# Nuralamsiddik16/Ultrafnd_git

Hardware: AMD Instinct MI355X
Metric: train-step samples/sec (FakeSV batch, seq128+224^2) (higher is better)
Workload: dtype bf16

## Files before the change

ultrafnd_git_amd/csrc/attn_softmax.hpp:

```cpp
#pragma once
#include "common.hpp"

#pragma clang fp contract(off)

__device__ __forceinline__ bf16x8 lds_frag(const char* tile, int row, int chunk) {
  return *reinterpret_cast<const bf16x8*>(tile + row * 128 + ((chunk ^ ((row >> 1) & 7)) << 4));
}

__device__ __forceinline__ bool masked_block_is_noop(const float* kb, int lane, const float (&m_run)[2]) {
  return __all(kb[lane] != 0.0f) && __all(m_run[0] > -1.0e30f && m_run[1] > -1.0e30f);
}

template <int KT, bool DROP = false, bool CAUSAL = false>
__device__ __forceinline__ float online_softmax_block(f32x4 (&s)[KT][2], const int qt, const float* kbias, const bool any_masked, const int g,
                                                      const float scale_log2e, float& m_run, float& l_run, bf16x8 (&pf)[KT / 2][2],
                                                      const f32x4* dm = nullptr, const int qk = 0, const float causal_neg = 0.0f) {
  float mx = -INFINITY, lsum = 0.0f, m_new, alpha;
  if (any_masked) {
#pragma unroll
    for (int kt = 0; kt < KT; ++kt) {
      const f32x4 kbv = *reinterpret_cast<const f32x4*>(kbias + kt * 16 + 4 * g);
#pragma unroll
      for (int r = 0; r < 4; ++r) {
        float v = (kbv[r] == 0.0f) ? s[kt][qt][r] * scale_log2e : kbv[r];
        if constexpr (CAUSAL) {
          if (kbv[r] == 0.0f && 16 * kt + r > qk) v = causal_neg;
        }
        s[kt][qt][r] = v;
        mx = fmaxf(mx, v);
      }
    }
    mx = fmaxf(mx, __shfl_xor(mx, 16, 64));
    mx = fmaxf(mx, __shfl_xor(mx, 32, 64));
    m_new = fmaxf(m_run, mx);
    alpha = fast_exp2(m_run - m_new);
#pragma unroll
    for (int kt = 0; kt < KT; ++kt)
#pragma unroll
      for (int r = 0; r < 4; ++r) {
        const float p = fast_exp2(s[kt][qt][r] - m_new);
        lsum += p;
        if constexpr (DROP) pf[kt >> 1][qt][(kt & 1) * 4 + r] = (__bf16)(p * dm[kt][r]);
        else pf[kt >> 1][qt][(kt & 1) * 4 + r] = (__bf16)p;
      }
  } else {
#pragma unroll
    for (int kt = 0; kt < KT; ++kt)
#pragma unroll
      for (int r = 0; r < 4; ++r) mx = fmaxf(mx, s[kt][qt][r]);
    mx = fmaxf(mx, __shfl_xor(mx, 16, 64));
    mx = fmaxf(mx, __shfl_xor(mx, 32, 64));
    m_new = fmaxf(m_run, mx * scale_log2e);
    alpha = fast_exp2(m_run - m_new);
    const float neg_m = -m_new;
#pragma unroll
    for (int kt = 0; kt < KT; ++kt)
#pragma unroll
      for (int r = 0; r < 4; ++r) {
        const float p = fast_exp2(__builtin_fmaf(s[kt][qt][r], scale_log2e, neg_m));
        lsum += p;
        if constexpr (DROP) pf[kt >> 1][qt][(kt & 1) * 4 + r] = (__bf16)(p * dm[kt][r]);
        else pf[kt >> 1][qt][(kt & 1) * 4 + r] = (__bf16)p;
      }
  }
  l_run = __builtin_fmaf(l_run, alpha, lsum);
  m_run = m_new;
  return alpha;
}

__device__ __forceinline__ void attn_init(f32x4 (&o)[4][2], float (&m_run)[2], float (&l_run)[2]) {
#pragma unroll
  for (int dt = 0; dt < 4; ++dt)
#pragma unroll
    for (int qt = 0; qt < 2; ++qt) o[dt][qt] = f32x4{0.f, 0.f, 0.f, 0.f};
#pragma unroll
  for (int qt = 0; qt < 2; ++qt) m_run[qt] = -INFINITY, l_run[qt] = 0.f;
}

template <class QRow>
__device__ __forceinline__ void attn_q_frags(const char* qimg, QRow q_row, int fr, int g, bf16x8 (&qf)[2][2]) {
#pragma unroll
  for (int qt = 0; qt < 2; ++qt) {
    const int row = q_row(qt * 16 + fr);
    qf[qt][0] = lds_frag(qimg, row, g);
    qf[qt][1] = lds_frag(qimg, row, g + 4);
  }
}

template <int KT, class KeyRow>
__device__ __forceinline__ void attn_scores(const char* kimg, KeyRow key_row, const bf16x8 (&qf)[2][2], int fr, int g, f32x4 (&s)[KT][2]) {
#pragma unroll
  for (int kt = 0; kt < KT; ++kt)
#pragma unroll
    for (int qt = 0; qt < 2; ++qt) s[kt][qt] = f32x4{0.f, 0.f, 0.f, 0.f};
#pragma unroll
  for (int kk = 0; kk < 2; ++kk)
#pragma unroll
    for (int kt = 0; kt < KT; ++kt) {
      const bf16x8 kf = lds_frag(kimg, key_row(kt * 16 + fr), g + 4 * kk);
#pragma unroll
      for (int qt = 0; qt < 2; ++qt) s[kt][qt] = __builtin_amdgcn_mfma_f32_16x16x32_bf16(kf, qf[qt][kk], s[kt][qt], 0, 0, 0);
    }
}

template <int KT, bool DROP = false, bool CAUSAL = false>
__device__ __forceinline__ void attn_softmax_rescale(f32x4 (&s)[KT][2], const int qt, const float* kbias, const bool any_masked, const int g,
                                                     const float scale_log2e, float (&m_run)[2], float (&l_run)[2], bf16x8 (&pf)[KT / 2][2],
                                                     f32x4 (&o)[4][2], const f32x4* dm = nullptr, const int qk = 0, const float causal_neg = 0.0f) {
  const float alpha = online_softmax_block<KT, DROP, CAUSAL>(s, qt, kbias, any_masked, g, scale_log2e, m_run[qt], l_run[qt], pf, dm, qk, causal_neg);
  if (!__all(alpha == 1.0f)) {
#pragma unroll
    for (int dt = 0; dt < 4; ++dt) o[dt][qt] *= alpha;
  }
}

template <int KT, class KeyRow>
__device__ __forceinline__ void attn_pv(const char* vimg, KeyRow key_row, const bf16x8 (&pf)[KT / 2][2], f32x4 (&o)[4][2], int fr, int g) {
#pragma unroll
  for (int ksd = 0; ksd < KT / 2; ++ksd) {
#pragma unroll
    for (int dt = 0; dt < 4; ++dt) {
      const int qq = fr >> 2, pp = fr & 3;
      const int k0 = 32 * ksd + 4 * g + qq;
      const int key0 = key_row(k0), key1 = key_row(k0 + 16);
      const int ch = 2 * dt + (pp >> 1);
      const int off0 = key0 * 128 + ((ch ^ (((key0 >> 1) & 3) << 1)) << 4) + 8 * (pp & 1);
      const int off1 = key1 * 128 + ((ch ^ (((key1 >> 1) & 3) << 1)) << 4) + 8 * (pp & 1);
      const s16x4 t0 = __builtin_amdgcn_ds_read_tr16_b64_v4i16((s16x4 __attribute__((address_space(3)))*)(vimg + off0));
      const s16x4 t1 = __builtin_amdgcn_ds_read_tr16_b64_v4i16((s16x4 __attribute__((address_space(3)))*)(vimg + off1));
      union { s16x4 s2[2]; bf16x8 v; } u;
      u.s2[0] = t0;
      u.s2[1] = t1;
#pragma unroll
      for (int qt = 0; qt < 2; ++qt) o[dt][qt] = __builtin_amdgcn_mfma_f32_16x16x32_bf16(u.v, pf[ksd][qt], o[dt][qt], 0, 0, 0);
    }
  }
}

__device__ __forceinline__ float attn_finish(const float l_run, float& l) {
  l = l_run;
  l += __shfl_xor(l, 16, 64);
  l += __shfl_xor(l, 32, 64);
  return 1.0f / l;
}
__device__ __forceinline__ float attn_finish(const float l_run) {
  float l;
  return attn_finish(l_run, l);
}

__device__ __forceinline__ void attn_store_ctx(__bf16* dst, const f32x4 (&o)[4][2], const int qt, const float inv) {
#pragma unroll
  for (int dt = 0; dt < 4; ++dt) {
    bf16x4 ov = {(__bf16)(o[dt][qt][0] * inv), (__bf16)(o[dt][qt][1] * inv), (__bf16)(o[dt][qt][2] * inv), (__bf16)(o[dt][qt][3] * inv)};
    *reinterpret_cast<bf16x4*>(dst + dt * 16) = ov;
  }
}
```

ultrafnd_git_amd/csrc/common.hpp:

```cpp
#pragma once
#include <hip/hip_runtime.h>
#include <stdint.h>
#include <stdio.h>

#include "../../include/ultrafnd_hip.h"

typedef float f32x16 __attribute__((ext_vector_type(16)));
typedef float f32x4 __attribute__((ext_vector_type(4)));
typedef float f32x2 __attribute__((ext_vector_type(2)));
typedef __bf16 bf16x8 __attribute__((ext_vector_type(8)));
typedef __bf16 bf16x4 __attribute__((ext_vector_type(4)));
typedef short s16x4 __attribute__((ext_vector_type(4)));

#define UFND_WAVE 64

void ufnd_set_error(const char* fmt, ...);
#define UFND_REQUIRE(cond, ...)                      \
  do {                                               \
    if (!(cond)) {                                   \
      ufnd_set_error(__VA_ARGS__);                   \
      return UFND_ERR_INVALID;                       \
    }                                                \
  } while (0)
#define UFND_CHECK_LAUNCH()                                              \
  do {                                                                   \
    hipError_t e_ = hipGetLastError();                                   \
    if (e_ != hipSuccess) {                                              \
      ufnd_set_error("%s:%d launch failed: %s", __FILE__, __LINE__,      \
                     hipGetErrorString(e_));                             \
      return UFND_ERR_LAUNCH;                                            \
    }                                                                    \
  } while (0)

static inline bool ufnd_aligned(const void* p, size_t a) { return (reinterpret_cast<uintptr_t>(p) % a) == 0; }
static inline int ufnd_cdiv(int a, int b) { return (a + b - 1) / b; }

__device__ __forceinline__ float gelu_f(float x) {
  return 0.5f * x * (1.0f + erff(x * 0.70710678118654752440f));
}
__device__ __forceinline__ float gelu_grad_f(float x) {
  const float cdf = 0.5f * (1.0f + erff(x * 0.70710678118654752440f));
  const float pdf = 0.39894228040143267794f * __expf(-0.5f * x * x);
  return cdf + x * pdf;
}
__device__ __forceinline__ float sigmoid_f(float x) { return 1.0f / (1.0f + __expf(-x)); }
__device__ __forceinline__ int xcd_contiguous_id(int n, int total) {
  const int q = total >> 3, r = total & 7, xcd = n & 7, idx = n >> 3;
  return (xcd < r ? xcd * (q + 1) : r * (q + 1) + (xcd - r) * q) + idx;
}

__device__ __forceinline__ float fast_exp2(float x) { return __builtin_amdgcn_exp2f(x); }
__device__ __forceinline__ float quick_gelu_grad_f(float x) {
  const float s = 1.0f / (1.0f + __expf(-1.702f * x));
  return s * (1.0f + 1.702f * x * (1.0f - s));
}
__device__ __forceinline__ float sigmoid_fast_f(float x) {
#pragma clang fp contract(off)
  return __builtin_amdgcn_rcpf(__fadd_rn(1.0f, __expf(-x)));
}
__device__ __forceinline__ float quick_gelu_fast_f(float x) {
#pragma clang fp contract(off)
  return __fmul_rn(x, sigmoid_fast_f(__fmul_rn(1.702f, x)));
}
__device__ __forceinline__ float gelu_fast_f(float x) {
#pragma clang fp contract(off)
  const float z = __fmul_rn(fabsf(x), 0.70710678118654752440f);
  const float t = __builtin_amdgcn_rcpf(__fmaf_rn(0.3275911f, z, 1.0f));
  float p = __fmaf_rn(t, 1.061405429f, -1.453152027f);
  p = __fmaf_rn(t, p, 1.421413741f);
  p = __fmaf_rn(t, p, -0.284496736f);
  p = __fmaf_rn(t, p, 0.254829592f);
  const float poly = __fmul_rn(t, p);
  const float erf_abs = __fmaf_rn(-poly, __expf(__fmul_rn(-z, z)), 1.0f);
  const float h = __fmul_rn(0.5f, x);
  return __fmaf_rn(h, copysignf(erf_abs, x), h);
}

__device__ __forceinline__ f32x2 gelu_fast_f2(f32x2 x) {
#pragma clang fp contract(off)
  const f32x2 z = __builtin_elementwise_abs(x) * 0.70710678118654752440f;
  const f32x2 u = __builtin_elementwise_fma(f32x2{0.3275911f, 0.3275911f}, z, f32x2{1.0f, 1.0f});
  const f32x2 t = {__builtin_amdgcn_rcpf(u.x), __builtin_amdgcn_rcpf(u.y)};
  f32x2 p = __builtin_elementwise_fma(t, f32x2{1.061405429f, 1.061405429f}, f32x2{-1.453152027f, -1.453152027f});
  p = __builtin_elementwise_fma(t, p, f32x2{1.421413741f, 1.421413741f});
  p = __builtin_elementwise_fma(t, p, f32x2{-0.284496736f, -0.284496736f});
  p = __builtin_elementwise_fma(t, p, f32x2{0.254829592f, 0.254829592f});
  const f32x2 poly = t * p;
  const f32x2 zz = (-z) * z;
  const f32x2 e = {__expf(zz.x), __expf(zz.y)};
  const f32x2 erf_abs = __builtin_elementwise_fma(-poly, e, f32x2{1.0f, 1.0f});
  const f32x2 h = x * 0.5f;
  const f32x2 sg = {copysignf(erf_abs.x, x.x), copysignf(erf_abs.y, x.y)};
  return __builtin_elementwise_fma(h, sg, h);
}
__device__ __forceinline__ f32x2 quick_gelu_fast_f2(f32x2 x) {
#pragma clang fp contract(off)
  const f32x2 m = x * 1.702f;
  const f32x2 d = f32x2{__expf(-m.x), __expf(-m.y)} + 1.0f;
  const f32x2 r = {__builtin_amdgcn_rcpf(d.x), __builtin_amdgcn_rcpf(d.y)};
  return x * r;
}

__device__ __forceinline__ float quad_xor1(float v) {
  return __builtin_bit_cast(float, __builtin_amdgcn_update_dpp(0, __builtin_bit_cast(int, v), 0xB1, 0xF, 0xF, false));
}
__device__ __forceinline__ float quad_xor2(float v) {
  return __builtin_bit_cast(float, __builtin_amdgcn_update_dpp(0, __builtin_bit_cast(int, v), 0x4E, 0xF, 0xF, false));
}

#define UFND_DPP(v, old, ctrl, rmask) \
  __builtin_bit_cast(float, __builtin_amdgcn_update_dpp(__builtin_bit_cast(int, (float)(old)), __builtin_bit_cast(int, (float)(v)), ctrl, rmask, 0xF, false))
__device__ __forceinline__ float wave_sum(float v) {
  v += UFND_DPP(v, 0.0f, 0xB1, 0xF);
  v += UFND_DPP(v, 0.0f, 0x4E, 0xF);
  v += UFND_DPP(v, 0.0f, 0x141, 0xF);
  v += UFND_DPP(v, 0.0f, 0x140, 0xF);
  v += UFND_DPP(v, 0.0f, 0x142, 0xA);
  v += UFND_DPP(v, 0.0f, 0x143, 0xC);
  return __builtin_bit_cast(float, __builtin_amdgcn_readlane(__builtin_bit_cast(int, v), 63));
}
__device__ __forceinline__ float wave_max(float v) {
  v = fmaxf(v, UFND_DPP(v, v, 0xB1, 0xF));
  v = fmaxf(v, UFND_DPP(v, v, 0x4E, 0xF));
  v = fmaxf(v, UFND_DPP(v, v, 0x141, 0xF));
  v = fmaxf(v, UFND_DPP(v, v, 0x140, 0xF));
  v = fmaxf(v, UFND_DPP(v, v, 0x142, 0xA));
  v = fmaxf(v, UFND_DPP(v, v, 0x143, 0xC));
  return __builtin_bit_cast(float, __builtin_amdgcn_readlane(__builtin_bit_cast(int, v), 63));
}

__device__ __forceinline__ void philox_4x32(uint64_t seed, uint64_t step, uint32_t layer, uint32_t ctr, uint32_t (&out)[4]) {
  uint32_t k0 = (uint32_t)seed, k1 = (uint32_t)(seed >> 32);
  uint32_t c0 = ctr, c1 = layer, c2 = (uint32_t)step, c3 = (uint32_t)(step >> 32);
#pragma unroll
  for (int r = 0; r < 10; ++r) {
    const uint64_t p0 = (uint64_t)0xD2511F53u * c0;
    const uint64_t p1 = (uint64_t)0xCD9E8D57u * c2;
    const uint32_t n0 = (uint32_t)(p1 >> 32) ^ c1 ^ k0;
    const uint32_t n1 = (uint32_t)p1;
    const uint32_t n2 = (uint32_t)(p0 >> 32) ^ c3 ^ k1;
    const uint32_t n3 = (uint32_t)p0;
    c0 = n0; c1 = n1; c2 = n2; c3 = n3;
    k0 += 0x9E3779B9u; k1 += 0xBB67AE85u;
  }
  out[0] = c0; out[1] = c1; out[2] = c2; out[3] = c3;
}
__device__ __forceinline__ float dropout_keep(uint32_t r, float p) {
  const float u = (float)(r >> 8) * (1.0f / 16777216.0f);
  return (u >= p) ? 1.0f / (1.0f - p) : 0.0f;
}
__device__ __forceinline__ uint64_t dropout_step_key(const ufnd_step_state* st) { return st->step + ((uint64_t)st->micro << 40); }
__device__ __forceinline__ float dropout_mul(const ufnd_step_state* st, float p, uint32_t layer, uint32_t elem) {
  if (p <= 0.0f) return 1.0f;
  uint32_t w[4];
  philox_4x32(st->seed, dropout_step_key(st), layer, elem >> 2, w);
  const uint32_t k = elem & 3u;
  return dropout_keep(k == 0 ? w[0] : (k == 1 ? w[1] : (k == 2 ? w[2] : w[3])), p);
}
__device__ __forceinline__ void dropout_mul4(const ufnd_step_state* st, float p, uint32_t layer, uint32_t elem4, float (&m)[4]) {
  if (p <= 0.0f) { m[0] = m[1] = m[2] = m[3] = 1.0f; return; }
  uint32_t w[4];
  philox_4x32(st->seed, dropout_step_key(st), layer, elem4 >> 2, w);
#pragma unroll
  for (int q = 0; q < 4; ++q) m[q] = dropout_keep(w[q], p);
}
__device__ __forceinline__ void dropout_mul4_ctr(uint64_t seed, uint64_t step, float p, uint32_t layer, uint32_t ctr, float (&m)[4]) {
  uint32_t w[4];
  philox_4x32(seed, step, layer, ctr, w);
#pragma unroll
  for (int q = 0; q < 4; ++q) m[q] = dropout_keep(w[q], p);
}

static inline bool ufnd_attn_dropout_fits(int B, int L, int heads) {
  const long long lp = (L + 3) / 4 * 4;
  return (long long)B * heads * L * lp / 4 <= (1ll << 32);
}
constexpr uint32_t UFND_TAG_TEXT = 256;
constexpr uint32_t UFND_TAG_VISION = 4096;
```

ultrafnd_git_amd/csrc/encoders.hip:

```cpp
#include "rowwise.hpp"

namespace {

template <int NI>
__global__ __launch_bounds__(256) void layernorm_kernel(const float* x, int ldx, const float* gamma, const float* beta,
                                                        __bf16* ob, float* of, int M, int H, float eps, const int* m_live) {
  const int lane = threadIdx.x & 63;
  const int row = blockIdx.x * 4 + (threadIdx.x >> 6);
  if (row >= M || (m_live && row >= *m_live)) return;
  f32x4 v[NI];
#pragma unroll
  for (int i = 0; i < NI; ++i) v[i] = ld4(x + (size_t)row * ldx + 4 * lane + 256 * i);
  ln_row<NI>(v, H, eps, gamma, beta, lane);
  store_row<NI>(v, ob, of, row, H, lane);
}

template <int NI, bool RESID>
__global__ __launch_bounds__(256) void dropout_layernorm_kernel(const float* x, int ldx, const float* d, int ldd, const float* gamma,
                                                                const float* beta, float* y, __bf16* ob, float* of, int M, int H, float eps,
                                                                ufnd_dropout dr) {
  const int lane = threadIdx.x & 63;
  const int row = blockIdx.x * 4 + (threadIdx.x >> 6);
  if (row >= M) return;
  const uint64_t seed = dr.state->seed, step = dropout_step_key(dr.state);
  f32x4 v[NI], m[NI];
#pragma unroll
  for (int i = 0; i < NI; ++i) {
    const int col = 4 * lane + 256 * i;
    float m4[4];
    dropout_mul4_ctr(seed, step, dr.p, dr.tag, (uint32_t)(((size_t)row * H + col) >> 2), m4);
    m[i] = f32x4{m4[0], m4[1], m4[2], m4[3]};
    v[i] = ld4(x + (size_t)row * ldx + col);
    if constexpr (RESID) {
      v[i] += m[i] * ld4(d + (size_t)row * ldd + col);
      *reinterpret_cast<f32x4*>(y + (size_t)row * H + col) = v[i];
    }
  }
  ln_row<NI>(v, H, eps, gamma, beta, lane);
  if constexpr (!RESID) {
#pragma unroll
    for (int i = 0; i < NI; ++i) v[i] *= m[i];
  }
  store_row<NI>(v, ob, of, row, H, lane);
}

template <int NI>
__global__ __launch_bounds__(256) void bert_embed_kernel(const int64_t* ids, const float* word, const float* pos,
                                                         const float* type0, const float* gamma, const float* beta,
                                                         __bf16* ob, float* of, int M, int L, int H, int vocab,
                                                         float eps, const int32_t* row_src, const int* m_live) {
  const int lane = threadIdx.x & 63;
  const int row = blockIdx.x * 4 + (threadIdx.x >> 6);
  if (row >= M || (m_live && row >= *m_live)) return;
  const int src = row_src ? row_src[row] : row;
  long long id = ids[src];
  id = id < 0 ? 0 : (id >= vocab ? vocab - 1 : id);
  int l = src % L;
  l = l < 0 ? 0 : (l >= L ? L - 1 : l);
  f32x4 v[NI];
#pragma unroll
  for (int i = 0; i < NI; ++i) {
    const int col = 4 * lane + 256 * i;
    v[i] = ld4(word + (size_t)id * H + col) + ld4(pos + (size_t)l * H + col) + ld4(type0 + col);
  }
  if (gamma) ln_row<NI>(v, H, eps, gamma, beta, lane);
  store_row<NI>(v, ob, of, row, H, lane);
}

template <bool PACKED>
__global__ __launch_bounds__(256) void meanpool_kernel(const float* hidden, const int32_t* mask, float* out, int L, int H, const int32_t* cu) {
  __shared__ f32x4 part[4][64];
  __shared__ float cnts[4];
  const int b = blockIdx.y, col = blockIdx.x * 256 + 4 * (threadIdx.x & 63), grp = threadIdx.x >> 6, lane = threadIdx.x & 63;
  f32x4 acc = {0.f, 0.f, 0.f, 0.f};
  float cnt = 0.0f;
  const size_t r0 = PACKED ? (size_t)cu[b] : (size_t)b * L;
  const int n = PACKED ? cu[b + 1] - cu[b] : L;
  for (int l0 = grp; l0 < n; l0 += 32) {
    int mk[8];
    f32x4 x[8];
#pragma unroll
    for (int u = 0; u < 8; ++u) {
      const int l = l0 + 4 * u;
      mk[u] = l < n ? mask[(size_t)b * L + l] : 0;
    }
#pragma unroll
    for (int u = 0; u < 8; ++u) {
      const int l = l0 + 4 * u < n ? l0 + 4 * u : n - 1;
      x[u] = ld4(hidden + (r0 + l) * H + col);
    }
#pragma unroll
    for (int u = 0; u < 8; ++u) {
      if (mk[u] != 0) {
        acc += x[u];
        cnt += 1.0f;
      }
    }
  }
  part[grp][lane] = acc;
  if (lane == 0) cnts[grp] = cnt;
  __syncthreads();
  if (grp == 0) {
    const f32x4 s = (part[0][lane] + part[1][lane]) + (part[2][lane] + part[3][lane]);
    const float denom = fmaxf((cnts[0] + cnts[1]) + (cnts[2] + cnts[3]), 1e-6f);
    *reinterpret_cast<f32x4*>(out + (size_t)b * H + col) = s / denom;
  }
}
template <int NI>
__global__ __launch_bounds__(256) void ln_meanpool_kernel(const float* y, const float* gamma, const float* beta, float eps, const int32_t* mask,
                                                          const int32_t* cu, float* out, int L, int H) {
  __shared__ f32x4 part[4][NI][64];
  __shared__ float cnts[4];
  const int b = blockIdx.x, grp = __builtin_amdgcn_readfirstlane(threadIdx.x >> 6), lane = threadIdx.x & 63;
  const size_t r0 = (size_t)cu[b];
  const int n = cu[b + 1] - cu[b];
  f32x4 acc[NI];
#pragma unroll
  for (int i = 0; i < NI; ++i) acc[i] = f32x4{0.f, 0.f, 0.f, 0.f};
  float cnt = 0.0f;
  for (int l0 = grp; l0 < n; l0 += 32) {
    int mk[8];
    f32x4 v[8][NI];
#pragma unroll
    for (int u = 0; u < 8; ++u) {
      const int l = l0 + 4 * u;
      mk[u] = l < n ? mask[(size_t)b * L + l] : 0;
    }
#pragma unroll
    for (int u = 0; u < 8; ++u) {
      const int l = l0 + 4 * u < n ? l0 + 4 * u : n - 1;
#pragma unroll
      for (int i = 0; i < NI; ++i) v[u][i] = ld4(y + (r0 + l) * H + 4 * lane + 256 * i);
    }
#pragma unroll
    for (int u = 0; u < 8; ++u) ln_row<NI>(v[u], H, eps, gamma, beta, lane);
#pragma unroll
    for (int u = 0; u < 8; ++u) {
      if (mk[u] != 0) {
#pragma unroll
        for (int i = 0; i < NI; ++i) acc[i] += v[u][i];
        cnt += 1.0f;
      }
    }
  }
#pragma unroll
  for (int i = 0; i < NI; ++i) part[grp][i][lane] = acc[i];
  if (lane == 0) cnts[grp] = cnt;
  __syncthreads();
  if (grp == 0) {
    const float denom = fmaxf((cnts[0] + cnts[1]) + (cnts[2] + cnts[3]), 1e-6f);
#pragma unroll
    for (int i = 0; i < NI; ++i) {
      const f32x4 s = (part[0][i][lane] + part[1][i][lane]) + (part[2][i][lane] + part[3][i][lane]);
      *reinterpret_cast<f32x4*>(out + (size_t)b * H + 4 * lane + 256 * i) = s / denom;
    }
  }
}

__device__ __forceinline__ void pack_slot_bins(const int* lens, int total, int B, int32_t* bins, int32_t* nbins) {
  __shared__ long long csum[PACK_THREADS / 64];
  const int tid = threadIdx.x, wave = tid >> 6, lane = tid & 63;
  const int per = (B + PACK_THREADS - 1) / PACK_THREADS, b0 = tid * per, b1 = min(b0 + per, B);
  auto nrows = [&](int b) { return (b + 1 < B ? lens[b + 1] : total) - lens[b]; };
  long long cown = 0;
  for (int b = b0; b < b1; ++b) {
    const int c = (nrows(b) + 31) >> 5;
    if (c > 0) cown += 1ll << (16 * (c - 1));
  }
  long long cinc = cown;
#pragma unroll
  for (int o = 1; o < 64; o <<= 1) {
    const long long y = __shfl_up(cinc, o, 64);
    if (lane >= o) cinc += y;
  }
  if (lane == 63) csum[wave] = cinc;
  __syncthreads();
  long long cbase = 0, call = 0;
  for (int w = 0; w < PACK_THREADS / 64; ++w) {
    if (w < wave) cbase += csum[w];
    call += csum[w];
  }
  auto field = [](long long v, int c) { return (int)((v >> (16 * (c - 1))) & 0xffff); };
  const int n1 = field(call, 1), n2 = field(call, 2), n3 = field(call, 3), n4 = field(call, 4);
  const int p = min(n1, n3), r1 = n1 - p, h = n2 >> 1, t = n2 & 1, u = t ? min(2, r1) : 0;
  const bool odd_full = t && u == 2;
  const int f1 = (r1 - u) >> 2, rem1 = (r1 - u) & 3;
  const int b31 = n4, b22 = b31 + p, b211 = b22 + h, b1111 = b211 + (odd_full ? 1 : 0);
  const int bp3 = b1111 + f1, bp2 = bp3 + (n3 - p), bp1 = bp2 + ((t && !odd_full) ? 1 : 0), nb = bp1 + (rem1 ? 1 : 0);
  const int bodd = odd_full ? b211 : bp2;
  long long rank = cbase + cinc - cown;
  for (int b = b0; b < b1; ++b) {
    const int n = nrows(b), c = (n + 31) >> 5;
    if (c == 0) continue;
    const int k = field(rank, c);
    rank += 1ll << (16 * (c - 1));
    int bin, s0;
    if (c == 4) {
      bin = k, s0 = 0;
    } else if (c == 3) {
      bin = k < p ? b31 + k : bp3 + (k - p), s0 = 0;
    } else if (c == 2) {
      bin = k < 2 * h ? b22 + (k >> 1) : bodd, s0 = k < 2 * h ? 2 * (k & 1) : 0;
    } else if (k < p) {
      bin = b31 + k, s0 = 3;
    } else if (k - p < u) {
      bin = bodd, s0 = 2 + (k - p);
    } else {
      const int k1 = k - p - u;
      bin = (k1 >> 2) < f1 ? b1111 + (k1 >> 2) : bp1, s0 = k1 & 3;
    }
    for (int s = 0; s < c; ++s) {
      bins[(size_t)bin * 8 + 2 * (s0 + s)] = lens[b] + 32 * s;
      bins[(size_t)bin * 8 + 2 * (s0 + s) + 1] = (b << 10) | (s << 8) | n;
    }
  }
  for (int i = bp3 + tid; i < nb; i += PACK_THREADS) {
    const int used = i < bp2 ? 3 : (i < bp1 ? 2 + u : rem1);
    for (int j = used; j < 4; ++j) {
      bins[(size_t)i * 8 + 2 * j] = 0;
      bins[(size_t)i * 8 + 2 * j + 1] = -1;
    }
  }
  if (tid == 0) *nbins = nb;
}

__global__ __launch_bounds__(PACK_THREADS) void text_pack_kernel(const int32_t* mask, int B, int L, int32_t* cu, int32_t* row_src,
                                                                 int32_t* bins, int32_t* nbins) {
  __shared__ int lens[PACK_MAX_B];
  const int tid = threadIdx.x, wave = tid >> 6, lane = tid & 63;
  for (int b = wave; b < B; b += PACK_THREADS / 64) {
    int last = 0;
    for (int l = lane; l < L; l += 64) last = mask[(size_t)b * L + l] != 0 ? l + 1 : last;
#pragma unroll
    for (int o = 32; o >= 1; o >>= 1) last = max(last, __shfl_xor(last, o, 64));
    if (lane == 0) lens[b] = last;
  }
  const int total = pack_scan_rows(lens, B, L, cu, row_src);
  if (bins) pack_slot_bins(lens, total, B, bins, nbins);
}

constexpr int TILE_MAX_B = UFND_TEXT_TILE_MAX_B, TILE_CAP = UFND_TEXT_TILE_SAMPLES, TILE_INTS = UFND_TEXT_TILE_INTS, TILE_MAX = TILE_MAX_B / 2;
__global__ __launch_bounds__(PACK_THREADS) void text_pack_tiles_kernel(const int32_t* mask, int B, int L, int32_t* cu, int32_t* row_src,
                                                                       int32_t* tiles, int32_t* ntiles, int32_t* bins, int32_t* nbins) {
  __shared__ int lens[TILE_MAX_B], order[TILE_MAX_B], place[TILE_MAX_B];
  __shared__ __attribute__((aligned(16))) int nb[TILE_MAX_B];
  __shared__ int t_rows[TILE_MAX], t_cnt[TILE_MAX], t_cu0[TILE_MAX];
  __shared__ unsigned char t_n[TILE_MAX * TILE_CAP];
  __shared__ unsigned long long kept[TILE_MAX_B][2];
  __shared__ int nlive_s, nt_s;
  const int tid = threadIdx.x, wave = tid >> 6, lane = tid & 63;
  if (tid == 0) nlive_s = 0;
  if (tid >= B && tid < TILE_MAX_B) nb[tid] = 0;
  constexpr int NWV = PACK_THREADS / 64;
  for (int b0 = wave; b0 < B; b0 += 4 * NWV) {
    int v[4][2];
#pragma unroll
    for (int j = 0; j < 4; ++j)
#pragma unroll
      for (int h = 0; h < 2; ++h) {
        const int b = b0 + NWV * j, l = lane + 64 * h;
        v[j][h] = (b < B && l < L) ? mask[(size_t)b * L + l] : 0;
      }
#pragma unroll
    for (int j = 0; j < 4; ++j) {
      const int b = b0 + NWV * j;
      if (b >= B) break;
      const unsigned long long m0 = __ballot(v[j][0] != 0), m1 = __ballot(v[j][1] != 0);
      const int last = m1 ? 128 - __clzll((long long)m1) : (m0 ? 64 - __clzll((long long)m0) : 0);
      if (lane == 0) {
        lens[b] = last;
        nb[b] = last;
        kept[b][0] = m0;
        kept[b][1] = m1;
      }
    }
  }
  const int total = pack_scan_rows(lens, B, L, cu, row_src);
  if (bins) pack_slot_bins(lens, total, B, bins, nbins);
  if (tid < B && nb[tid] > 0) {
    const int n = nb[tid];
    int rank = 0;
#pragma unroll 4
    for (int b = 0; b < B; b += 4) {
      const int4 v = *reinterpret_cast<const int4*>(nb + b);
      rank += (v.x > n || (v.x == n && b < tid)) + (v.y > n || (v.y == n && b + 1 < tid)) + (v.z > n || (v.z == n && b + 2 < tid)) +
              (v.w > n || (v.w == n && b + 3 < tid));
    }
    order[rank] = tid;
    atomicAdd(&nlive_s, 1);
  }
  __syncthreads();
  const int nl = nlive_s;
  if (wave == 0) {
    int st[TILE_MAX / 64], key[TILE_MAX / 64];
#pragma unroll
    for (int c = 0; c < TILE_MAX / 64; ++c) { st[c] = 0; key[c] = 256; }
    for (int i0 = 0; nl <= 128 && i0 < nl; i0 += 64) {
      const int vn = i0 + lane < nl ? nb[order[i0 + lane]] : 0;
      const int cnt = min(64, nl - i0);
      int s0 = st[0], k0 = key[0];
      for (int j = 0; j < cnt; ++j) {
        const int n = __builtin_amdgcn_readlane(vn, j);
        const bool mine = lane == __ffsll((long long)__ballot(k0 >= n)) - 1;
        if (mine) place[i0 + j] = (lane << 12) | ((s0 >> 16) << 8) | (s0 & 0xffff);
        s0 += mine ? (1 << 16) + n : 0;
        k0 = s0 < (TILE_CAP << 16) ? 256 - (s0 & 0xffff) : -1;
      }
      st[0] = s0;
      key[0] = k0;
    }
    for (int i0 = 0; nl > 128 && i0 < nl; i0 += 64) {
      const int vn = i0 + lane < nl ? nb[order[i0 + lane]] : 0;
      const int cnt = min(64, nl - i0);
      int pv = 0;
      for (int j = 0; j < cnt; ++j) {
        const int n = __builtin_amdgcn_readlane(vn, j);
        bool placed = false;
#pragma unroll
        for (int c = 0; c < TILE_MAX / 64; ++c) {
          const unsigned long long m = placed ? 0ull : __ballot(key[c] >= n);
          if (m == 0) continue;
          const int l = __ffsll((long long)m) - 1;
          const int was = __builtin_amdgcn_readlane(st[c], l);
          pv = lane == j ? ((64 * c + l) << 12) | ((was >> 16) << 8) | (was & 0xffff) : pv;
          st[c] += lane == l ? (1 << 16) + n : 0;
          key[c] = st[c] < (TILE_CAP << 16) ? 256 - (st[c] & 0xffff) : -1;
          placed = true;
        }
      }
      if (i0 + lane < nl) place[i0 + lane] = pv;
    }
    int nt = 0;
#pragma unroll
    for (int c = 0; c < TILE_MAX / 64; ++c) {
      nt += __popcll(__ballot(st[c] != 0));
      t_rows[64 * c + lane] = st[c] & 0xffff;
      t_cnt[64 * c + lane] = st[c] >> 16;
    }
    if (lane == 0) {
      nt_s = nt;
      *ntiles = nt;
    }
  }
  __syncthreads();
  const int nt = nt_s;
  if (tid < nl) {
    const int b = order[tid], p = place[tid], t = p >> 12, slot = (p >> 8) & 15, r0 = p & 255;
    tiles[(size_t)t * TILE_INTS + 4 + 2 * slot] = lens[b];
    tiles[(size_t)t * TILE_INTS + 5 + 2 * slot] = (b << 16) | (r0 << 8) | nb[b];
    t_n[t * TILE_CAP + slot] = (unsigned char)nb[b];
    if (slot == 0) t_cu0[t] = lens[b];
  }
  for (int i = wave; i < nl; i += NWV) {
    const int b = order[i], n = nb[b], p = place[i], r0 = p & 255, row0 = lens[b];
    int32_t* td = tiles + (size_t)(p >> 12) * TILE_INTS;
#pragma unroll
    for (int h = 0; h < 2; ++h) {
      const int k = lane + 64 * h;
      if (k >= n) continue;
      td[UFND_TEXT_TILE_ROWMAP + r0 + k] = row0 + k;
      td[UFND_TEXT_TILE_KBIAS + r0 + k] = __float_as_int(((kept[b][h] >> lane) & 1) ? 0.0f : -3.0e38f);
    }
  }
  __syncthreads();
  if (tid < nt) {
    int32_t* td = tiles + (size_t)tid * TILE_INTS;
    const int cnt = t_cnt[tid];
    int u = 0;
    for (int j = 0; j < cnt; ++j)
      for (int q = 0; q < (t_n[tid * TILE_CAP + j] + 31) >> 5; ++q) td[UFND_TEXT_TILE_UNIT0 + u++] = j | (q << 8);
    td[0] = cnt;
    td[1] = t_rows[tid];
    td[2] = u;
    td[3] = 0;
  }
  for (int idx = tid; idx < nt * 256; idx += PACK_THREADS) {
    const int t = idx >> 8, r = idx & 255;
    if (r < t_rows[t]) continue;
    tiles[(size_t)t * TILE_INTS + UFND_TEXT_TILE_ROWMAP + r] = t_cu0[t];
    tiles[(size_t)t * TILE_INTS + UFND_TEXT_TILE_KBIAS + r] = __float_as_int(-3.0e38f);
  }
}

__global__ __launch_bounds__(256) void l2norm_rows_kernel(float* x, int H) {
  __shared__ float sh[4];
  float* row = x + (size_t)blockIdx.x * H;
  float sq = 0.0f;
  for (int c = threadIdx.x; c < H; c += 256) sq += row[c] * row[c];
  sq = wave_sum(sq);
  if ((threadIdx.x & 63) == 0) sh[threadIdx.x >> 6] = sq;
  __syncthreads();
  const float nrm = sqrtf((sh[0] + sh[1]) + (sh[2] + sh[3])) + 1e-9f;
  for (int c = threadIdx.x; c < H; c += 256) row[c] = row[c] / nrm;
}

template <int PT, int GT>
__global__ __launch_bounds__(256) void patchify_kernel(const float* frames, __bf16* patches, int S_, int P_) {
  const int P = PT ? PT : P_, G = GT ? GT : S_ / P_, S = P * G;
  const int n = blockIdx.x / G, py = blockIdx.x - n * G;
  const int K = 3 * P * P, CPR = P / 8;
  const int chunks = 3 * P * G * CPR;
  const float* src = frames + ((size_t)n * 3 * S + (size_t)py * P) * S;
  __bf16* dst = patches + ((size_t)n * G * G + (size_t)py * G) * K;
  for (int q = threadIdx.x; q < chunks; q += 256) {
    const int x8 = q % (G * CPR), r = q / (G * CPR);
    const int ky = r % P, c = r / P;
    const int px = x8 / CPR, kx = (x8 - px * CPR) * 8;
    const float* sp = src + ((size_t)c * S + ky) * S + x8 * 8;
    const f32x4 v0 = ld4(sp), v1 = ld4(sp + 4);
    bf16x8 o = {(__bf16)v0[0], (__bf16)v0[1], (__bf16)v0[2], (__bf16)v0[3], (__bf16)v1[0], (__bf16)v1[1], (__bf16)v1[2], (__bf16)v1[3]};
    *reinterpret_cast<bf16x8*>(dst + (size_t)px * K + c * P * P + ky * P + kx) = o;
  }
}

template <int NI>
__global__ __launch_bounds__(256) void vit_assemble_kernel(const float* pe, const float* cls, const float* pos,
                                                           const float* gamma, const float* beta, float* of, __bf16* ob,
                                                           float* stats, int M, int P, int H, float eps) {
  const int lane = threadIdx.x & 63;
  const int row = blockIdx.x * 4 + (threadIdx.x >> 6);
  if (row >= M) return;
  const int n = row / (P + 1), t = row % (P + 1);
  f32x4 v[NI];
#pragma unroll
  for (int i = 0; i < NI; ++i) {
    const int col = 4 * lane + 256 * i;
    const f32x4 base = (t == 0) ? ld4(cls + col) : ld4(pe + ((size_t)n * P + (t - 1)) * H + col);
    v[i] = base + ld4(pos + (size_t)t * H + col);
  }
  if (gamma) ln_row<NI>(v, H, eps, gamma, beta, lane);
  store_row<NI>(v, ob, of, row, H, lane);
  if (stats) row_stats<NI>(v, stats, row, lane);
}

__global__ __launch_bounds__(256) void l2norm_frames_kernel(const float* e, float* out, int F, int D) {
  __shared__ float sh[4];
  const int b = blockIdx.x;
  float acc[4] = {0, 0, 0, 0};
  for (int f = 0; f < F; ++f) {
    const float* row = e + ((size_t)b * F + f) * D;
    float sq = 0.0f;
    for (int c = threadIdx.x; c < D; c += 256) sq += row[c] * row[c];
    const float nrm = sqrtf(block_sum4(sq, sh)) + 1e-9f;
    int n = 0;
    for (int c = threadIdx.x; c < D; c += 256, ++n) acc[n] += row[c] / nrm;
  }
  if (F == 1) {
    int n = 0;
    for (int c = threadIdx.x; c < D; c += 256, ++n) out[(size_t)b * D + c] = acc[n];
    return;
  }
  float sq = 0.0f;
  int n = 0;
  for (int c = threadIdx.x; c < D; c += 256, ++n) {
    acc[n] /= (float)F;
    sq += acc[n] * acc[n];
  }
  const float nrm = sqrtf(block_sum4(sq, sh)) + 1e-9f;
  n = 0;
  for (int c = threadIdx.x; c < D; c += 256, ++n) out[(size_t)b * D + c] = acc[n] / nrm;
}

__global__ __launch_bounds__(256) void field_mean_l2_kernel(const float* parts, const int32_t* valid, float* out, int Mx,
                                                            int D) {
  __shared__ float sh[4];
  const int n = blockIdx.x;
  float acc[4] = {0, 0, 0, 0};
  int cnt = 0;
  for (int m = 0; m < Mx; ++m) {
    if (valid[(size_t)n * Mx + m] == 0) continue;
    ++cnt;
    const float* row = parts + ((size_t)n * Mx + m) * D;
    int k = 0;
    for (int c = threadIdx.x; c < D; c += 256, ++k) acc[k] += row[c];
  }
  float sq = 0.0f;
  int k = 0;
  for (int c = threadIdx.x; c < D; c += 256, ++k) {
    acc[k] = cnt ? acc[k] / (float)cnt : 0.0f;
    sq += acc[k] * acc[k];
  }
  sq = wave_sum(sq);
  if ((threadIdx.x & 63) == 0) sh[threadIdx.x >> 6] = sq;
  __syncthreads();
  const float nrm = sqrtf((sh[0] + sh[1]) + (sh[2] + sh[3])) + 1e-9f;
  k = 0;
  for (int c = threadIdx.x; c < D; c += 256, ++k) out[(size_t)n * D + c] = cnt ? acc[k] / nrm : 0.0f;
}

}

extern "C" int ufnd_layernorm(const float* x, int ldx, const float* gamma, const float* beta, void* out_bf16,
                              float* out_f32, int M, int H, float eps, void* stream_) {
  UFND_REQUIRE(x && gamma && beta && (out_bf16 || out_f32) && M >= 1, "layernorm: null argument");
  UFND_REQUIRE(h_ok(H), "layernorm: H=%d (supported 256/512/768/1024)", H);
  UFND_REQUIRE(ldx % 4 == 0 && ldx >= H && ufnd_aligned(x, 16) && ufnd_aligned(gamma, 16) && ufnd_aligned(beta, 16) &&
                   (!out_f32 || ufnd_aligned(out_f32, 16)) && (!out_bf16 || ufnd_aligned(out_bf16, 8)), "layernorm: alignment");
  NI_LAUNCH(H, layernorm_kernel, dim3(ufnd_cdiv(M, 4)), (hipStream_t)stream_, x, ldx, gamma, beta, (__bf16*)out_bf16,
            out_f32, M, H, eps, (const int*)nullptr);
  UFND_CHECK_LAUNCH();
  return UFND_OK;
}

extern "C" int ufnd_dropout_residual_layernorm(const float* x, int ldx, const float* d, int ldd, const float* gamma, const float* beta, float* y,
                                               void* out_bf16, float* out_f32, int M, int H, float eps, const ufnd_dropout* drop, void* stream_) {
  UFND_REQUIRE(x && d && gamma && beta && y && (out_bf16 || out_f32) && M >= 1 && drop && drop->state, "dropout_residual_layernorm: null argument");
  UFND_REQUIRE(drop->p > 0.0f && drop->p < 1.0f, "dropout_residual_layernorm: p=%g (0 < p < 1)", (double)drop->p);
  UFND_REQUIRE(h_ok(H), "dropout_residual_layernorm: H=%d (supported 256/512/768/1024)", H);
  UFND_REQUIRE(ldx % 4 == 0 && ldx >= H && ldd % 4 == 0 && ldd >= H && ufnd_aligned(x, 16) && ufnd_aligned(d, 16) && ufnd_aligned(y, 16) &&
                   ufnd_aligned(gamma, 16) && ufnd_aligned(beta, 16) && (!out_f32 || ufnd_aligned(out_f32, 16)) && (!out_bf16 || ufnd_aligned(out_bf16, 8)),
               "dropout_residual_layernorm: alignment");
  UFND_REQUIRE((long long)M * H / 4 <= (1ll << 32), "dropout_residual_layernorm: M=%d H=%d overflows the 32-bit dropout counter", M, H);
  NI_LAUNCH_T(H, dropout_layernorm_kernel, true, dim3(ufnd_cdiv(M, 4)), (hipStream_t)stream_, x, ldx, d, ldd, gamma, beta, y, (__bf16*)out_bf16,
            out_f32, M, H, eps, *drop);
  UFND_CHECK_LAUNCH();
  return UFND_OK;
}

extern "C" int ufnd_layernorm_dropout(const float* x, int ldx, const float* gamma, const float* beta, void* out_bf16, float* out_f32, int M, int H,
                                      float eps, const ufnd_dropout* drop, void* stream_) {
  UFND_REQUIRE(x && gamma && beta && (out_bf16 || out_f32) && M >= 1 && drop && drop->state, "layernorm_dropout: null argument");
  UFND_REQUIRE(drop->p > 0.0f && drop->p < 1.0f, "layernorm_dropout: p=%g (0 < p < 1)", (double)drop->p);
  UFND_REQUIRE(h_ok(H), "layernorm_dropout: H=%d (supported 256/512/768/1024)", H);
  UFND_REQUIRE(ldx % 4 == 0 && ldx >= H && ufnd_aligned(x, 16) && ufnd_aligned(gamma, 16) && ufnd_aligned(beta, 16) &&
                   (!out_f32 || ufnd_aligned(out_f32, 16)) && (!out_bf16 || ufnd_aligned(out_bf16, 8)), "layernorm_dropout: alignment");
  UFND_REQUIRE((long long)M * H / 4 <= (1ll << 32), "layernorm_dropout: M=%d H=%d overflows the 32-bit dropout counter", M, H);
  NI_LAUNCH_T(H, dropout_layernorm_kernel, false, dim3(ufnd_cdiv(M, 4)), (hipStream_t)stream_, x, ldx, (const float*)nullptr, 0, gamma, beta,
            (float*)nullptr, (__bf16*)out_bf16, out_f32, M, H, eps, *drop);
  UFND_CHECK_LAUNCH();
  return UFND_OK;
}

extern "C" int ufnd_bert_embed(const int64_t* ids, const float* word, const float* pos, const float* type0,
                               const float* gamma, const float* beta, void* x_bf16, float* x_f32, int B, int L, int H,
                               int vocab, float eps, void* stream_) {
  UFND_REQUIRE(ids && word && pos && type0 && ((gamma && beta) || (!gamma && !beta)) && (x_bf16 || x_f32), "bert_embed: null argument");
  UFND_REQUIRE(h_ok(H) && B >= 1 && L >= 1 && vocab >= 1, "bert_embed: B=%d L=%d H=%d vocab=%d", B, L, H, vocab);
  UFND_REQUIRE(ufnd_aligned(word, 16) && ufnd_aligned(pos, 16) && ufnd_aligned(type0, 16) &&
                   (!x_f32 || ufnd_aligned(x_f32, 16)) && (!x_bf16 || ufnd_aligned(x_bf16, 8)), "bert_embed: alignment");
  const int M = B * L;
  NI_LAUNCH(H, bert_embed_kernel, dim3(ufnd_cdiv(M, 4)), (hipStream_t)stream_, ids, word, pos, type0, gamma, beta,
            (__bf16*)x_bf16, x_f32, M, L, H, vocab, eps, (const int32_t*)nullptr, (const int*)nullptr);
  UFND_CHECK_LAUNCH();
  return UFND_OK;
}

extern "C" int ufnd_masked_meanpool(const float* hidden, const int32_t* mask, float* out, int B, int L, int H, void* stream_) {
  UFND_REQUIRE(hidden && mask && out, "meanpool: null argument");
  UFND_REQUIRE(B >= 1 && B <= 65535 && L >= 1, "meanpool: B=%d L=%d (1 <= B <= 65535 clips, L >= 1 rows)", B, L);
  UFND_REQUIRE(H >= 256 && H % 256 == 0 && ufnd_aligned(hidden, 16) && ufnd_aligned(out, 16), "meanpool: H=%d (multiple of 256)", H);
  hipLaunchKernelGGL(meanpool_kernel<false>, dim3(H / 256, B), dim3(256), 0, (hipStream_t)stream_, hidden, mask, out, L, H,
                     (const int32_t*)nullptr);
  UFND_CHECK_LAUNCH();
  return UFND_OK;
}

extern "C" int ufnd_masked_meanpool_l2(const float* hidden, const int32_t* mask, float* out, int B, int L, int H,
                                       void* stream_) {
  UFND_REQUIRE(hidden && mask && out && B >= 1 && L >= 1, "meanpool: null argument");
  UFND_REQUIRE(H >= 256 && H % 256 == 0 && ufnd_aligned(hidden, 16) && ufnd_aligned(out, 16), "meanpool: H=%d (multiple of 256)", H);
  hipLaunchKernelGGL(meanpool_kernel<false>, dim3(H / 256, B), dim3(256), 0, (hipStream_t)stream_, hidden, mask, out, L, H,
                     (const int32_t*)nullptr);
  UFND_CHECK_LAUNCH();
  hipLaunchKernelGGL(l2norm_rows_kernel, dim3(B), dim3(256), 0, (hipStream_t)stream_, out, H);
  UFND_CHECK_LAUNCH();
  return UFND_OK;
}

extern "C" int ufnd_text_pack(const int32_t* mask, int B, int L, int32_t* cu_seqlens, int32_t* row_src, void* stream_) {
  UFND_REQUIRE(mask && cu_seqlens && row_src, "text_pack: null argument");
  UFND_REQUIRE(B >= 1 && B <= PACK_MAX_B && L >= 1 && (long long)B * L < (1ll << 31), "text_pack: B=%d L=%d (B <= %d)", B, L, PACK_MAX_B);
  hipLaunchKernelGGL(text_pack_kernel, dim3(1), dim3(PACK_THREADS), 0, (hipStream_t)stream_, mask, B, L, cu_seqlens, row_src,
                     (int32_t*)nullptr, (int32_t*)nullptr);
  UFND_CHECK_LAUNCH();
  return UFND_OK;
}

extern "C" int ufnd_text_pack_bins(const int32_t* mask, int B, int L, int32_t* cu_seqlens, int32_t* row_src, int32_t* bins,
                                   int32_t* nbins, void* stream_) {
  UFND_REQUIRE(mask && cu_seqlens && row_src && bins && nbins, "text_pack_bins: null argument");
  UFND_REQUIRE(B >= 1 && B <= PACK_MAX_B && L >= 1 && L <= 128, "text_pack_bins: B=%d L=%d (B <= %d, L <= 128)", B, L, PACK_MAX_B);
  hipLaunchKernelGGL(text_pack_kernel, dim3(1), dim3(PACK_THREADS), 0, (hipStream_t)stream_, mask, B, L, cu_seqlens, row_src, bins, nbins);
  UFND_CHECK_LAUNCH();
  return UFND_OK;
}

extern "C" int ufnd_text_pack_tiles(const int32_t* mask, int B, int L, int32_t* cu_seqlens, int32_t* row_src, int32_t* tiles,
                                    int32_t* ntiles, int32_t* bins, int32_t* nbins, void* stream_) {
  UFND_REQUIRE(mask && cu_seqlens && row_src && tiles && ntiles && !bins == !nbins, "text_pack_tiles: null argument");
  UFND_REQUIRE(B >= 1 && B <= TILE_MAX_B && L >= 1 && L <= 128, "text_pack_tiles: B=%d L=%d (B <= %d, L <= 128)", B, L, TILE_MAX_B);
  hipLaunchKernelGGL(text_pack_tiles_kernel, dim3(1), dim3(PACK_THREADS), 0, (hipStream_t)stream_, mask, B, L, cu_seqlens, row_src, tiles, ntiles,
                     bins, nbins);
  UFND_CHECK_LAUNCH();
  return UFND_OK;
}

extern "C" int ufnd_bert_embed_live(const int64_t* ids, const int32_t* row_src, const int* m_live, const float* word, const float* pos,
                                    const float* type0, const float* gamma, const float* beta, void* x_bf16, float* x_f32, int capacity,
                                    int L, int H, int vocab, float eps, void* stream_) {
  UFND_REQUIRE(ids && row_src && m_live && word && pos && type0 && gamma && beta && (x_bf16 || x_f32), "bert_embed_live: null argument");
  UFND_REQUIRE(h_ok(H) && capacity >= 1 && L >= 1 && vocab >= 1, "bert_embed_live: capacity=%d L=%d H=%d vocab=%d", capacity, L, H, vocab);
  UFND_REQUIRE(ufnd_aligned(word, 16) && ufnd_aligned(pos, 16) && ufnd_aligned(type0, 16) &&
                   (!x_f32 || ufnd_aligned(x_f32, 16)) && (!x_bf16 || ufnd_aligned(x_bf16, 8)), "bert_embed_live: alignment");
  NI_LAUNCH(H, bert_embed_kernel, dim3(ufnd_cdiv(capacity, 4)), (hipStream_t)stream_, ids, word, pos, type0, gamma, beta,
            (__bf16*)x_bf16, x_f32, capacity, L, H, vocab, eps, row_src, m_live);
  UFND_CHECK_LAUNCH();
  return UFND_OK;
}

extern "C" int ufnd_layernorm_live(const float* x, int ldx, const float* gamma, const float* beta, void* out_bf16, float* out_f32,
                                   int capacity, int H, float eps, const int* m_live, void* stream_) {
  UFND_REQUIRE(x && gamma && beta && (out_bf16 || out_f32) && m_live && capacity >= 1, "layernorm_live: null argument");
  UFND_REQUIRE(h_ok(H), "layernorm_live: H=%d (supported 256/512/768/1024)", H);
  UFND_REQUIRE(ldx % 4 == 0 && ldx >= H && ufnd_aligned(x, 16) && ufnd_aligned(gamma, 16) && ufnd_aligned(beta, 16) &&
                   (!out_f32 || ufnd_aligned(out_f32, 16)) && (!out_bf16 || ufnd_aligned(out_bf16, 8)), "layernorm_live: alignment");
  NI_LAUNCH(H, layernorm_kernel, dim3(ufnd_cdiv(capacity, 4)), (hipStream_t)stream_, x, ldx, gamma, beta, (__bf16*)out_bf16,
            out_f32, capacity, H, eps, m_live);
  UFND_CHECK_LAUNCH();
  return UFND_OK;
}

extern "C" int ufnd_masked_meanpool_l2_live(const float* hidden, const int32_t* mask, const int32_t* cu_seqlens, float* out, int B, int L,
                                            int H, void* stream_) {
  UFND_REQUIRE(hidden && mask && cu_seqlens && out && B >= 1 && L >= 1, "meanpool_live: null argument");
  UFND_REQUIRE(H >= 256 && H % 256 == 0 && ufnd_aligned(hidden, 16) && ufnd_aligned(out, 16), "meanpool_live: H=%d (multiple of 256)", H);
  hipLaunchKernelGGL(meanpool_kernel<true>, dim3(H / 256, B), dim3(256), 0, (hipStream_t)stream_, hidden, mask, out, L, H, cu_seqlens);
  UFND_CHECK_LAUNCH();
  hipLaunchKernelGGL(l2norm_rows_kernel, dim3(B), dim3(256), 0, (hipStream_t)stream_, out, H);
  UFND_CHECK_LAUNCH();
  return UFND_OK;
}

extern "C" int ufnd_ln_masked_meanpool_l2_live(const float* y, const float* gamma, const float* beta, float eps, const int32_t* mask,
                                               const int32_t* cu_seqlens, float* out, int B, int L, int H, void* stream_) {
  UFND_REQUIRE(y && gamma && beta && mask && cu_seqlens && out && B >= 1 && L >= 1, "ln_meanpool_live: null argument");
  UFND_REQUIRE(h_ok(H), "ln_meanpool_live: H=%d (supported 256/512/768/1024)", H);
  UFND_REQUIRE(ufnd_aligned(y, 16) && ufnd_aligned(gamma, 16) && ufnd_aligned(beta, 16) && ufnd_aligned(out, 16), "ln_meanpool_live: alignment");
  NI_LAUNCH(H, ln_meanpool_kernel, dim3(B), (hipStream_t)stream_, y, gamma, beta, eps, mask, cu_seqlens, out, L, H);
  UFND_CHECK_LAUNCH();
  hipLaunchKernelGGL(l2norm_rows_kernel, dim3(B), dim3(256), 0, (hipStream_t)stream_, out, H);
  UFND_CHECK_LAUNCH();
  return UFND_OK;
}

extern "C" int ufnd_vit_patchify(const float* frames, void* patches, int N, int image, int patch, void* stream_) {
  UFND_REQUIRE(frames && patches && N >= 1, "patchify: null argument");
  UFND_REQUIRE(patch % 8 == 0 && image % patch == 0 && ufnd_aligned(frames, 16) && ufnd_aligned(patches, 16),
               "patchify: image=%d patch=%d (patch a multiple of 8, 16-B aligned buffers)", image, patch);
  const int G = image / patch;
  if (patch == 32 && G == 7) hipLaunchKernelGGL((patchify_kernel<32, 7>), dim3(N * G), dim3(256), 0, (hipStream_t)stream_, frames, (__bf16*)patches, image, patch);
  else hipLaunchKernelGGL((patchify_kernel<0, 0>), dim3(N * G), dim3(256), 0, (hipStream_t)stream_, frames, (__bf16*)patches, image, patch);
  UFND_CHECK_LAUNCH();
  return UFND_OK;
}

extern "C" int ufnd_vit_assemble(const float* patch_emb, const float* cls, const float* pos, const float* gamma,
                                 const float* beta, float* x_f32, void* x_bf16, float* stats, int N, int P, int H, float eps,
                                 void* stream_) {
  UFND_REQUIRE(patch_emb && cls && pos && ((gamma && beta) || (!gamma && !beta)) && (x_f32 || x_bf16) && N >= 1 && P >= 1, "vit_assemble: null argument");
  UFND_REQUIRE(h_ok(H), "vit_assemble: H=%d", H);
  const int M = N * (P + 1);
  UFND_REQUIRE(!stats || ufnd_aligned(stats, 16), "vit_assemble: stats alignment");
  UFND_REQUIRE((!x_f32 || ufnd_aligned(x_f32, 16)) && (!x_bf16 || ufnd_aligned(x_bf16, 8)), "vit_assemble: alignment");
  NI_LAUNCH(H, vit_assemble_kernel, dim3(ufnd_cdiv(M, 4)), (hipStream_t)stream_, patch_emb, cls, pos, gamma, beta, x_f32,
            (__bf16*)x_bf16, stats, M, P, H, eps);
  UFND_CHECK_LAUNCH();
  return UFND_OK;
}

extern "C" int ufnd_l2norm_frames(const float* e, float* out, int B, int F, int D, void* stream_) {
  UFND_REQUIRE(e && out && B >= 1 && F >= 1 && D >= 1 && D <= 1024, "l2norm_frames: B=%d F=%d D=%d", B, F, D);
  hipLaunchKernelGGL(l2norm_frames_kernel, dim3(B), dim3(256), 0, (hipStream_t)stream_, e, out, F, D);
  UFND_CHECK_LAUNCH();
  return UFND_OK;
}

extern "C" int ufnd_field_mean_l2(const float* parts, const int32_t* valid, float* out, int N, int Mx, int D, void* stream_) {
  UFND_REQUIRE(parts && valid && out && N >= 1 && Mx >= 1 && D >= 1 && D <= 1024, "field_mean_l2: N=%d M=%d D=%d", N, Mx, D);
  hipLaunchKernelGGL(field_mean_l2_kernel, dim3(N), dim3(256), 0, (hipStream_t)stream_, parts, valid, out, Mx, D);
  UFND_CHECK_LAUNCH();
  return UFND_OK;
}

namespace {
__global__ __launch_bounds__(256) void ln_fold_guard_kernel(const float* stats, int M, int parts, float inv_h, float eps, float* guard) {
  __shared__ float sh[4];
  float worst = 0.0f;
  const int nq = parts >> 1, sub = threadIdx.x & 3;
  const long long total = M;
  const long long step = (long long)gridDim.x * 64;
  for (long long r = (long long)blockIdx.x * 64 + (threadIdx.x >> 2); r < total; r += 2 * step) {
    f32x4 v[2][3];
    bool live[2];
#pragma unroll
    for (int k = 0; k < 2; ++k) {
      const long long rk = r + k * step;
      live[k] = rk < total;
      const long long rc = live[k] ? rk : r;
      const f32x4* p = reinterpret_cast<const f32x4*>(stats + (size_t)rc * parts * 2);
#pragma unroll
      for (int u = 0; u < 3; ++u) {
        const int c = sub + 4 * u;
        v[k][u] = p[c < nq ? c : sub];
      }
    }
#pragma unroll
    for (int k = 0; k < 2; ++k) {
      float sm = 0.0f, sq = 0.0f;
#pragma unroll
      for (int u = 0; u < 3; ++u) {
        if (sub + 4 * u < nq) {
          sm += v[k][u][0] + v[k][u][2];
          sq += v[k][u][1] + v[k][u][3];
        }
      }
      sm += quad_xor1(sm); sq += quad_xor1(sq);
      sm += quad_xor2(sm); sq += quad_xor2(sq);
      const float mean = sm * inv_h;
      const float var = fmaxf(sq * inv_h - mean * mean, 0.0f);
      if (live[k]) {
        float ratio = fabsf(mean) * rsqrtf(var + eps);
        ratio = ratio == ratio ? ratio : INFINITY;
        worst = fmaxf(worst, ratio);
      }
    }
  }
  worst = wave_max(worst);
  if ((threadIdx.x & 63) == 0) sh[threadIdx.x >> 6] = worst;
  __syncthreads();
  if (threadIdx.x == 0)
    atomicMax(reinterpret_cast<int*>(guard), __float_as_int(fmaxf(fmaxf(sh[0], sh[1]), fmaxf(sh[2], sh[3]))));
}
}

extern "C" int ufnd_ln_fold_guard(const float* stats, int M, int parts, int width, float eps, float* guard, void* stream_) {
  UFND_REQUIRE(stats && guard && M >= 1 && parts >= 2 && parts <= 24 && parts % 2 == 0 && width >= 1 && ufnd_aligned(stats, 16),
               "ln_fold_guard: M=%d parts=%d (even)", M, parts);
  const int want = (int)((M + 63ll) / 64);
  hipLaunchKernelGGL(ln_fold_guard_kernel, dim3(want < 2048 ? want : 2048), dim3(256), 0, (hipStream_t)stream_, stats, M, parts,
                     1.0f / (float)width, eps, guard);
  UFND_CHECK_LAUNCH();
  return UFND_OK;
}
```

Measured before the change: 29610.

## Use permlane swaps for cross-row reductions and closed-form placement of long samples

Replaces the __shfl_xor by 16 and 32 in the attention softmax max and sum reductions with permlane16/permlane32 swap intrinsics, avoiding LDS-backed bpermute. In the text tile packing kernel, samples longer than a third of a tile are placed in closed form, two per tile, and only the remaining samples go through the serial first-fit wave loop. This shortens the sequential placement scan but adds a lane-id select per swap. A diagnostic kernel is added to check lane-partner equivalence.

New measurement: 29650 (median of 3 runs). About the same (+0.1%).

```diff
diff --git a/ultrafnd_git_amd/csrc/attn_softmax.hpp b/ultrafnd_git_amd/csrc/attn_softmax.hpp
--- a/ultrafnd_git_amd/csrc/attn_softmax.hpp
+++ b/ultrafnd_git_amd/csrc/attn_softmax.hpp
@@ -30,8 +30,8 @@
         mx = fmaxf(mx, v);
       }
     }
-    mx = fmaxf(mx, __shfl_xor(mx, 16, 64));
-    mx = fmaxf(mx, __shfl_xor(mx, 32, 64));
+    mx = fmaxf(mx, lane_xor16(mx));
+    mx = fmaxf(mx, lane_xor32(mx));
     m_new = fmaxf(m_run, mx);
     alpha = fast_exp2(m_run - m_new);
 #pragma unroll
@@ -48,8 +48,8 @@
     for (int kt = 0; kt < KT; ++kt)
 #pragma unroll
       for (int r = 0; r < 4; ++r) mx = fmaxf(mx, s[kt][qt][r]);
-    mx = fmaxf(mx, __shfl_xor(mx, 16, 64));
-    mx = fmaxf(mx, __shfl_xor(mx, 32, 64));
+    mx = fmaxf(mx, lane_xor16(mx));
+    mx = fmaxf(mx, lane_xor32(mx));
     m_new = fmaxf(m_run, mx * scale_log2e);
     alpha = fast_exp2(m_run - m_new);
     const float neg_m = -m_new;
@@ -139,8 +139,8 @@
 
 __device__ __forceinline__ float attn_finish(const float l_run, float& l) {
   l = l_run;
-  l += __shfl_xor(l, 16, 64);
-  l += __shfl_xor(l, 32, 64);
+  l += lane_xor16(l);
+  l += lane_xor32(l);
   return 1.0f / l;
 }
 __device__ __forceinline__ float attn_finish(const float l_run) {
diff --git a/ultrafnd_git_amd/csrc/common.hpp b/ultrafnd_git_amd/csrc/common.hpp
--- a/ultrafnd_git_amd/csrc/common.hpp
+++ b/ultrafnd_git_amd/csrc/common.hpp
@@ -107,6 +107,17 @@
 __device__ __forceinline__ float quad_xor2(float v) {
   return __builtin_bit_cast(float, __builtin_amdgcn_update_dpp(0, __builtin_bit_cast(int, v), 0x4E, 0xF, 0xF, false));
 }
+__device__ __forceinline__ int lane_id() { return (int)__builtin_amdgcn_mbcnt_hi(~0u, __builtin_amdgcn_mbcnt_lo(~0u, 0u)); }
+__device__ __forceinline__ float lane_xor16(float v) {
+  const unsigned u = __builtin_bit_cast(unsigned, v);
+  const auto r = __builtin_amdgcn_permlane16_swap(u, u, false, false);
+  return __builtin_bit_cast(float, (lane_id() & 16) ? r[0] : r[1]);
+}
+__device__ __forceinline__ float lane_xor32(float v) {
+  const unsigned u = __builtin_bit_cast(unsigned, v);
+  const auto r = __builtin_amdgcn_permlane32_swap(u, u, false, false);
+  return __builtin_bit_cast(float, (lane_id() & 32) ? r[0] : r[1]);
+}
 
 #define UFND_DPP(v, old, ctrl, rmask) \
   __builtin_bit_cast(float, __builtin_amdgcn_update_dpp(__builtin_bit_cast(int, (float)(old)), __builtin_bit_cast(int, (float)(v)), ctrl, rmask, 0xF, false))
diff --git a/ultrafnd_git_amd/csrc/diag/lane_partner.hip b/ultrafnd_git_amd/csrc/diag/lane_partner.hip
--- /dev/null
+++ b/ultrafnd_git_amd/csrc/diag/lane_partner.hip
@@ -0,0 +1,19 @@
+#include "../common.hpp"
+
+namespace {
+__global__ __launch_bounds__(64) void lane_partner_kernel(const float* in, float* out, int n) {
+  const int i = blockIdx.x * 64 + threadIdx.x;
+  const float v = in[i];
+  out[i] = lane_xor16(v);
+  out[64 * n + i] = lane_xor32(v);
+  out[128 * n + i] = __shfl_xor(v, 16, 64);
+  out[192 * n + i] = __shfl_xor(v, 32, 64);
+}
+}
+
+extern "C" int ufnd_diag_lane_partner(const float* in, float* out, int waves, void* stream) {
+  UFND_REQUIRE(in && out && waves >= 1 && waves <= 1024, "diag_lane_partner: bad argument");
+  hipLaunchKernelGGL(lane_partner_kernel, dim3(waves), dim3(64), 0, (hipStream_t)stream, in, out, waves);
+  UFND_CHECK_LAUNCH();
+  return UFND_OK;
+}
diff --git a/ultrafnd_git_amd/csrc/encoders.hip b/ultrafnd_git_amd/csrc/encoders.hip
--- a/ultrafnd_git_amd/csrc/encoders.hip
+++ b/ultrafnd_git_amd/csrc/encoders.hip
@@ -240,6 +240,8 @@
 }
 
 constexpr int TILE_MAX_B = UFND_TEXT_TILE_MAX_B, TILE_CAP = UFND_TEXT_TILE_SAMPLES, TILE_INTS = UFND_TEXT_TILE_INTS, TILE_MAX = TILE_MAX_B / 2;
+constexpr int TILE_BIG = 256 / 3;
+static_assert(3 * (TILE_BIG + 1) > 256 && TILE_CAP > 2, "the closed-form placement of the long samples");
 __global__ __launch_bounds__(PACK_THREADS) void text_pack_tiles_kernel(const int32_t* mask, int B, int L, int32_t* cu, int32_t* row_src,
                                                                        int32_t* tiles, int32_t* ntiles, int32_t* bins, int32_t* nbins) {
   __shared__ int lens[TILE_MAX_B], order[TILE_MAX_B], place[TILE_MAX_B];
@@ -247,9 +249,9 @@
   __shared__ int t_rows[TILE_MAX], t_cnt[TILE_MAX], t_cu0[TILE_MAX];
   __shared__ unsigned char t_n[TILE_MAX * TILE_CAP];
   __shared__ unsigned long long kept[TILE_MAX_B][2];
-  __shared__ int nlive_s, nt_s;
+  __shared__ int nlive_s, nbig_s, nt_s;
   const int tid = threadIdx.x, wave = tid >> 6, lane = tid & 63;
-  if (tid == 0) nlive_s = 0;
+  if (tid == 0) nlive_s = nbig_s = 0;
   if (tid >= B && tid < TILE_MAX_B) nb[tid] = 0;
   constexpr int NWV = PACK_THREADS / 64;
   for (int b0 = wave; b0 < B; b0 += 4 * NWV) {
@@ -288,14 +290,20 @@
     }
     order[rank] = tid;
     atomicAdd(&nlive_s, 1);
-  }
-  __syncthreads();
-  const int nl = nlive_s;
+    if (n > TILE_BIG) atomicAdd(&nbig_s, 1);
+  }
+  __syncthreads();
+  const int nl = nlive_s, nbig = nbig_s;
   if (wave == 0) {
     int st[TILE_MAX / 64], key[TILE_MAX / 64];
-#pragma unroll
-    for (int c = 0; c < TILE_MAX / 64; ++c) { st[c] = 0; key[c] = 256; }
-    for (int i0 = 0; nl <= 128 && i0 < nl; i0 += 64) {
+    for (int i = lane; i < nbig; i += 64) place[i] = ((i >> 1) << 12) | ((i & 1) << 8) | ((i & 1) ? nb[order[i - 1]] : 0);
+#pragma unroll
+    for (int c = 0; c < TILE_MAX / 64; ++c) {
+      const int i = 2 * (64 * c + lane);
+      st[c] = i + 1 < nbig ? (2 << 16) + nb[order[i]] + nb[order[i + 1]] : (i < nbig ? (1 << 16) + nb[order[i]] : 0);
+      key[c] = 256 - (st[c] & 0xffff);
+    }
+    for (int i0 = nbig; nl <= 128 && i0 < nl; i0 += 64) {
       const int vn = i0 + lane < nl ? nb[order[i0 + lane]] : 0;
       const int cnt = min(64, nl - i0);
       int s0 = st[0], k0 = key[0];
@@ -309,7 +317,7 @@
       st[0] = s0;
       key[0] = k0;
     }
-    for (int i0 = 0; nl > 128 && i0 < nl; i0 += 64) {
+    for (int i0 = nbig; nl > 128 && i0 < nl; i0 += 64) {
       const int vn = i0 + lane < nl ? nb[order[i0 + lane]] : 0;
       const int cnt = min(64, nl - i0);
       int pv = 0;
```
